# mkln/spamtree

Hardware: NVIDIA B200
Metric: mcmc_iterations_per_sec (higher is better)
Workload: dtype f64

## Files before the change

spamtree_b200/csrc/st_kernels.cu:

```cuda
#include <cuda_runtime.h>

#include <algorithm>
#include <cstdint>

#include "st_device.cuh"
#include "st_kernels.cuh"

namespace st {

__device__ __forceinline__ double iloo_term(double resid, double mean, double v, double tq) {
  const double s2 = v + 1.0 / tq, d = resid - mean;
  return -0.5 * (log(6.283185307179586 * s2) + d * d / s2);
}
template <int REF, bool ILOO>
__global__ void __launch_bounds__(kGibbsThreads)
gibbs_level_kernel(DevTree T, DevSlots D, int slot0, double* __restrict__ w, const double* __restrict__ xb,
                   const double* __restrict__ z, const double* __restrict__ tausq_inv, const double* __restrict__ SigS,
                   double* __restrict__ V, double* probe_sig, double* probe_smu, int* __restrict__ fail,
                   double* __restrict__ ll, const double* __restrict__ yobs) {
  extern __shared__ __align__(16) unsigned char smem_raw[];
  asm volatile("griddepcontrol.launch_dependents;");
  const DevSlot S = pick_slot(D, D.chain->cur);
  const int tid = threadIdx.x, nth = blockDim.x, lane = tid & 31, warp = tid >> 5;
  const int sd = slot0 + blockIdx.x;
  const int m = T.m[sd], k = T.k[sd], P = T.P[sd], coff = T.chain_off[sd], row0 = T.row0[sd];
  const int rsm = tile_rs(m), gs = T.gs[sd];
  const int msq = REF ? m * rsm : m;
  double* RiS = reinterpret_cast<double*>(smem_raw);
  double* Sig = RiS + msq;
  double* wpa = Sig + (REF ? m * m : m);
  double* gwj = wpa + P;
  double* smu = gwj + (size_t)(k + 1) * m;
  double* wn = smu + m;
  double* rr = wn + m;
  const double* G = S.G + T.goff[sd];
  const double* Rig = S.Ri + T.rioff[sd];
  const int nch = T.child_ptr[sd + 1] - T.child_ptr[sd];
  const int* ch = T.child_idx + T.child_ptr[sd];
  __shared__ int c_m[32], c_po[32], c_r0[32];
  __shared__ long long c_voff[16];
  __shared__ double cbuf[128];
  if (tid < k) {
    const int a = T.chain[coff + tid];
    c_m[tid] = T.m[a]; c_po[tid] = T.chain_poff[coff + tid]; c_r0[tid] = T.row0[a];
  }
  for (int c = tid; c < min(nch, 16); c += nth) c_voff[c] = T.voff[ch[c]];
  for (int e = tid; e < msq; e += nth) RiS[e] = Rig[e];
  if (REF) {
    const long long so0 = T.soff[sd];
    for (int e = tid; e < m * m; e += nth) Sig[e] = (so0 >= 0) ? SigS[so0 + e] : 0.0;
  }
  for (int a = tid; a < m; a += nth) {
    const double tq = tausq_inv[T.mvq[row0 + a]];
    wn[a] = tq;
    smu[a] = tq * (T.y[row0 + a] - xb[row0 + a]);
    rr[a] = z[row0 + a];
  }
  __syncthreads();
  for (int e = tid; e < P; e += nth) {
    int j = 0;
    while (j + 1 < k && e >= c_po[j + 1]) j++;
    wpa[e] = w[c_r0[j] + (e - c_po[j])];
  }
  __syncthreads();
  for (int e = tid; e < k * m; e += nth) {
    const int r = e / k, j = e - r * k;
    const int mj = c_m[j], po = c_po[j];
    const double* g = G + (size_t)r * gs + po;
    const double* wv = wpa + po;
    double s[4] = {0, 0, 0, 0};
    int pp = 0;
    for (; pp + 8 <= mj; pp += 8) {
      double x[8];
#pragma unroll
      for (int u = 0; u < 8; u++) x[u] = g[pp + u];
#pragma unroll
      for (int u = 0; u < 8; u++) s[u & 3] = fma(x[u], wv[pp + u], s[u & 3]);
    }
    if (pp + 4 <= mj) {
      double x[4];
#pragma unroll
      for (int u = 0; u < 4; u++) x[u] = g[pp + u];
#pragma unroll
      for (int u = 0; u < 4; u++) s[u] = fma(x[u], wv[pp + u], s[u]);
      pp += 4;
    }
    for (; pp < mj; pp++) s[0] = fma(g[pp], wv[pp], s[0]);
    gwj[j * m + r] = (s[0] + s[1]) + (s[2] + s[3]);
  }
  __syncthreads();
  for (int r = tid; r < m; r += nth) {
    double s = 0;
    for (int j = 0; j < k; j++) s += gwj[j * m + r];
    gwj[k * m + r] = s;
  }
  __syncthreads();
  const double* gw = gwj + (size_t)k * m;
  if (REF) {
    for (int e = tid; e < m * m; e += nth) {
      const int a = e / m, b = e - a * m;
      double s = 0;
      for (int r = max(a, b); r < m; r++) s = fma(RiS[r * rsm + a], RiS[r * rsm + b], s);
      s += Sig[e];
      if (a == b) s += wn[a];
      Sig[e] = s;
      if (probe_sig) probe_sig[T.rioff[sd] + e] = s;
    }
    __syncthreads();
    bool okc = true;
    double myinv = 0.0;
    if (warp == 0) {
      if (m <= 32) {
        double a[32];
#pragma unroll
        for (int j = 0; j < 32; j++) a[j] = (lane < m && j <= lane) ? Sig[lane * m + j] : 0.0;
        cbuf[32 + lane] = 0.0;
        cbuf[96 + lane] = 0.0;
        __syncwarp();
        for (int j = 0; j < m; j++) {
          double d = __shfl_sync(0xffffffffu, a[0], j);
          if (!(d > 0.0) || !isfinite(d)) { okc = false; d = 1.0; }
          const double inv = rsqrt(d), sd = d * inv;
          const double l = (lane == j) ? sd : ((lane > j) ? a[0] * inv : 0.0);
          if (lane == j) myinv = inv;
          if (lane >= j && lane < m) Sig[lane * m + j] = l;
          double* cc = cbuf + (j & 1) * 64;
          cc[lane] = l;
          __syncwarp();
          const double* cj = cc + j + 1;
#pragma unroll
          for (int i = 0; i < 31; i++) a[i] = fma(-l, cj[i], a[i + 1]);
          a[31] = 0.0;
        }
        __syncwarp();
      } else {
        okc = warp_chol(Sig, m, m, lane);
      }
    }
    asm volatile("griddepcontrol.wait;" ::: "memory");
    for (int a = tid; a < m; a += nth) {
      double s = 0;
      for (int r = a; r < m; r++) s = fma(RiS[r * rsm + a], gw[r], s);
      for (int c = 0; c < nch; c++) s += V[(c < 16 ? c_voff[c] : T.voff[ch[c]]) + (T.limited ? 0 : P) + a];
      s += smu[a];
      smu[a] = s;
      if (probe_smu) probe_smu[row0 + a] = s;
    }
    __syncthreads();
    if (warp == 0) {
      if (okc && m <= 32) {
        double b = (lane < m) ? smu[lane] : 0.0;
        for (int j = 0; j < m; j++) {
          const double xj = __shfl_sync(0xffffffffu, b * myinv, j);
          if (lane == j) b = xj; else if (lane > j && lane < m) b = fma(-Sig[lane * m + j], xj, b);
        }
        double y = (lane < m) ? b + rr[lane] : 0.0;
        for (int j = m - 1; j >= 0; j--) {
          const double wj = __shfl_sync(0xffffffffu, y * myinv, j);
          if (lane == j) y = wj; else if (lane < j) y = fma(-Sig[j * m + lane], wj, y);
        }
        if (lane < m) { wn[lane] = y; w[row0 + lane] = y; }
      } else if (okc) {
        for (int c = 0; c < m; c++) {
          __syncwarp();
          const double xc = smu[c] / Sig[c * m + c];
          __syncwarp();
          if (lane == 0) smu[c] = xc;
          for (int r = c + 1 + lane; r < m; r += 32) smu[r] -= Sig[r * m + c] * xc;
        }
        __syncwarp();
        for (int r = lane; r < m; r += 32) smu[r] += rr[r];
        for (int c = m - 1; c >= 0; c--) {
          __syncwarp();
          const double xc = smu[c] / Sig[c * m + c];
          __syncwarp();
          if (lane == 0) smu[c] = xc;
          for (int r = lane; r < c; r += 32) smu[r] -= Sig[c * m + r] * xc;
        }
        __syncwarp();
        for (int r = lane; r < m; r += 32) { wn[r] = smu[r]; w[row0 + r] = smu[r]; }
      }
      if (!okc) {
        if (lane == 0) atomicAdd(fail, 1);
        for (int r = lane; r < m; r += 32) wn[r] = w[row0 + r];
      }
    }
    __syncthreads();
    if (ILOO) {
      const long long so0 = T.soff[sd];
      const bool back = (m & 1) == 0;
      for (int a = tid; a < m; a += nth) {
        const int i = row0 + a;
        const double yi = yobs[i];
        if (isnan(yi)) continue;
        double lz = 0.0, qa = 0.0;
        for (int t = 0; t <= a; t++) {
          const int j = back ? a - t : t;
          lz = fma(Sig[a * m + j], rr[j], lz);
        }
        for (int r = a; r < m; r++) qa = fma(RiS[r * rsm + a], RiS[r * rsm + a], qa);
        if (so0 >= 0) qa += SigS[so0 + (long long)a * m + a];
        const double tq = tausq_inv[T.mvq[i]], res = yi - xb[i], wa = wn[a];
        ll[i] = iloo_term(res, wa - (lz + tq * (res - wa)) / qa, 1.0 / qa, tq);
      }
      __syncthreads();
    }
    for (int r = tid; r < m; r += nth) {
      double s = -gw[r];
      for (int r2 = 0; r2 <= r; r2++) s = fma(RiS[r * rsm + r2], wn[r2], s);
      rr[r] = s;
    }
  } else {
    asm volatile("griddepcontrol.wait;" ::: "memory");
    for (int a = tid; a < m; a += nth) {
      const double ri = RiS[a], prec = ri * ri;
      const double sig = prec + wn[a];
// ... 22 lines not shown
    int j = 0;
    while (j + 1 < k && e >= c_po[j + 1]) j++;
    const int rsj = gs;
    const double* g = G + e;
    const double* vj = gwj + (size_t)j * m;
    double sa[4] = {0, 0, 0, 0};
    int r = 0;
    for (; r + 8 <= m; r += 8) {
      double x[8];
#pragma unroll
      for (int u = 0; u < 8; u++) x[u] = g[(size_t)(r + u) * rsj];
#pragma unroll
      for (int u = 0; u < 8; u++) sa[u & 3] = fma(x[u], vj[r + u], sa[u & 3]);
    }
    if (r + 4 <= m) {
      double x[4];
#pragma unroll
      for (int u = 0; u < 4; u++) x[u] = g[(size_t)(r + u) * rsj];
#pragma unroll
      for (int u = 0; u < 4; u++) sa[u] = fma(x[u], vj[r + u], sa[u]);
      r += 4;
    }
    for (; r < m; r++) sa[0] = fma(g[(size_t)r * rsj], vj[r], sa[0]);
    double s = (sa[0] + sa[1]) + (sa[2] + sa[3]);
    if (!T.limited)
      for (int c = 0; c < nch; c++) s += V[(c < 16 ? c_voff[c] : T.voff[ch[c]]) + e];
    Vd[e] = s;
  }
}

cudaError_t launch_gibbs(int is_ref, const DevTree& T, const DevSlots& D, int slot0, int nslots, double* w,
                         const double* xb, const double* z, const double* tausq_inv, const double* SigS, double* V,
                         double* probe_sig, double* probe_smu, int* fail, size_t smem, cudaStream_t st, bool pdl, double* ll,
                         const double* yobs) {
  if (nslots <= 0) return cudaSuccess;
  static SmemOptIn optin[4];
  const bool iloo = ll != nullptr;
  auto kern = is_ref ? (iloo ? gibbs_level_kernel<1, true> : gibbs_level_kernel<1, false>)
                     : (iloo ? gibbs_level_kernel<0, true> : gibbs_level_kernel<0, false>);
  {
    cudaError_t e = ensure_dynamic_smem(kern, smem, optin[(is_ref ? 1 : 0) + (iloo ? 2 : 0)]);
    if (e != cudaSuccess) return e;
  }
  cudaLaunchConfig_t cfg = {};
  cfg.gridDim = dim3(nslots);
  cfg.blockDim = dim3(kGibbsThreads);
  cfg.dynamicSmemBytes = smem;
  cfg.stream = st;
  cudaLaunchAttribute attr[1];
  attr[0].id = cudaLaunchAttributeProgrammaticStreamSerialization;
  attr[0].val.programmaticStreamSerializationAllowed = 1;
  cfg.attrs = attr;
  cfg.numAttrs = pdl ? 1 : 0;
  return cudaLaunchKernelEx(&cfg, kern, T, D, slot0, w, xb, z, tausq_inv, SigS, V, probe_sig, probe_smu, fail, ll, yobs);
}

__global__ void __launch_bounds__(kGramThreads)
gram_level_kernel(DevTree T, DevSlots D, int slot0, double* __restrict__ U, double* __restrict__ SigS, int rch, int ldx,
                  int stage_off, const int* __restrict__ run_flag) {
  extern __shared__ __align__(16) double gram_smem[];
  asm volatile("griddepcontrol.launch_dependents;");
  if (run_flag != nullptr && *run_flag == 0) return;
  const DevSlot S = pick_slot(D, D.chain->cur);
  __shared__ int t_po[kMaxChain + 1], t_m[kMaxChain + 1], t_item0[kMaxChain + 2], t_uo[kMaxChain + 1], t_to[kMaxChain + 2];
  __shared__ int s_rows;
  __shared__ long long s_rowoff[kGramMaxRows];
  __shared__ int s_rowncol[kGramMaxRows];
  __shared__ long long s_cu[kGramChildTab];
  __shared__ int f_m[kGramFusedTab], f_gs[kGramFusedTab], f_r0[kGramFusedTab + 1];
  __shared__ long long f_goff[kGramFusedTab];
  const int tid = threadIdx.x, nth = blockDim.x;
  const int sd = slot0 + blockIdx.x;
  if (T.ufused[sd]) return;
  double* tiles = gram_smem;
  double* stage = gram_smem + stage_off;
  const int m = T.m[sd], k = T.k[sd], P = T.P[sd], coff = T.chain_off[sd];
  const int nch = T.child_ptr[sd + 1] - T.child_ptr[sd];
  const int* ch = T.child_idx + T.child_ptr[sd];
  const long long so = T.soff[sd];
  const int ntile = k + (so >= 0 ? 1 : 0);
  if (tid <= k) {
    t_po[tid] = (tid < k) ? T.chain_poff[coff + tid] : (T.limited ? 0 : P);
    t_m[tid] = (tid < k) ? T.m[T.chain[coff + tid]] : m;
    t_uo[tid] = (tid < k) ? T.chain_uoff[coff + tid] : 0;
  }
  const bool ftab = nch <= kGramFusedTab;
  if (ftab && tid < nch) {
// ... 1307 lines not shown
```

spamtree_b200/csrc/st_kernels.cuh:

```cuda
#pragma once
#include <cuda_runtime.h>

#include <cstddef>
#include <cstdint>

#include "st_build_plan.cuh"
#include "st_model.hpp"

namespace st {

constexpr int kGibbsThreads = 64;
constexpr int kGramThreads = 256;
constexpr int kGramMaxRows = 256;
constexpr int kGramChildTab = 256;
constexpr int kGramFusedTab = 64;
constexpr int kLlwThreads = 128;
constexpr int kLlwMaxP = 1024;
constexpr double kHl2pi = -0.91893853320467274178;

inline size_t gibbs_smem_bytes(int is_ref, int m, int P, int k) {
  const size_t msq = is_ref ? (size_t)m * tile_rs(m) + (size_t)m * m : 2 * (size_t)m;
  return 8 * (msq + (size_t)P + (size_t)(k + 1) * m + 3 * (size_t)m) + 16;
}

struct SmemOptIn { size_t configured[64] = {}; };
template <class K>
inline cudaError_t ensure_dynamic_smem(K kern, size_t smem, SmemOptIn& table) {
  int dev = 0;
  cudaError_t e = cudaGetDevice(&dev);
  if (e != cudaSuccess) return e;
  if (dev < 0 || dev >= 64) return cudaFuncSetAttribute(kern, cudaFuncAttributeMaxDynamicSharedMemorySize, (int)smem);
  if (smem <= table.configured[dev]) return cudaSuccess;
  e = cudaFuncSetAttribute(kern, cudaFuncAttributeMaxDynamicSharedMemorySize, (int)smem);
  if (e == cudaSuccess) table.configured[dev] = smem;
  return e;
}

cudaError_t launch_build(int mode, const DevTree& T, const DevSlots& D, int rel, double* predG, double* predRi, int want_H,
                         const int* grp_slot0, const int* grp_nn, int ngrp, const double* w, int* fail, int ns, int phase, size_t smem,
                         cudaStream_t st, int nthreads, unsigned long long* prof = nullptr, bool pdl = false,
                         const int* run_flag = nullptr);
cudaError_t launch_gibbs(int is_ref, const DevTree& T, const DevSlots& D, int slot0, int nslots, double* w,
                         const double* xb, const double* z, const double* tausq_inv, const double* SigS, double* V,
                         double* probe_sig, double* probe_smu, int* fail, size_t smem, cudaStream_t st, bool pdl = false,
                         double* ll = nullptr,
                         const double* yobs = nullptr);
cudaError_t launch_gram(const DevTree& T, const DevSlots& D, int slot0, int nslots, double* U, double* SigS, int rch,
                        int ldx, int tile_doubles, int stage_off, int threads, cudaStream_t st, const int* run_flag = nullptr,
                        bool pdl = false);
cudaError_t launch_llw(const DevTree& T, const DevSlots& D, int rel, int slot0, int nslots, const double* w, int maxlen, cudaStream_t st,
                       double* vrow = nullptr, int parked = 0);
constexpr int kReduceScratch = 4 * 32 + 2;
cudaError_t launch_loglik_reduce(const DevSlots& D, int rel, int n_top, int n, int* fail, double* out8, double* scratch,
                                 cudaStream_t st);
cudaError_t launch_frontier_sum(const DevTree& T, int n, const int* pseudo, const int* c0, const int* c1, const int* vlen,
                                const int* ulen, double* V, double* U, int do_v, int do_u, cudaStream_t st);
cudaError_t launch_predict_sample(const DevTree& T, int slot0, int nslots, const double* Hpred, const double* sdpred,
                                  double* w, const double* z, cudaStream_t st);
cudaError_t launch_normals(double* z, long long n, uint64_t seed, uint64_t counter, const long long* rowkey, const int* iter_ptr,
                           cudaStream_t st);
cudaError_t launch_rowstats(const DevTree& T, const int* widx, long long n_all, int p, int q, const double* w,
                            const double* xb, double* partial, int nblocks, double* out, cudaStream_t st);
cudaError_t launch_xb(const DevTree& T, long long n_all, int p, const double* bcoeff, double* xb, cudaStream_t st);
cudaError_t launch_permute(const double* src, double* dst, const long long* map, long long n, cudaStream_t st);
cudaError_t launch_crosscov(const double* x1, const double* y1, const int* q1, long long n1, const double* x2,
                            const double* y2, const int* q2, long long n2, const CovTab& tab, double* out,
                            cudaStream_t st);
cudaError_t launch_mh_propose(ChainDev* C, cudaStream_t st, int iter_offset = 0);
cudaError_t launch_mh_accept(ChainDev* C, int mode, int have_llw, cudaStream_t st, int npar = 0);
cudaError_t launch_predict_gate(ChainDev* C, cudaStream_t st);
cudaError_t launch_tausq_beta(ChainDev* C, const double* stats, const double* xtx, double* tausq_inv, double* bcoeff,
                              double* scratch, int sample_tausq, int sample_beta, cudaStream_t st, int p = 0, int q = 0);
cudaError_t launch_record(ChainDev* C, const double* tausq_inv, const double* bcoeff, double* theta_mcmc, double* beta_mcmc,
                          double* tausq_mcmc, int keep, cudaStream_t st, int tick = 0);
cudaError_t launch_yhat(const DevTree& T, const double* w, const double* xb, const double* tausq_inv, const long long* iperm,
                        const long long* rowkey, long long n, const ChainDev* C, double* out, cudaStream_t st);
cudaError_t launch_chain_tick(ChainDev* C, cudaStream_t st);
struct ThetaPack {
  int n;
// ... 41 lines not shown
```

spamtree_b200/csrc/st_model.cu:

```cuda
#include "st_model.hpp"

#include <algorithm>
#include <cmath>
#include <cstdlib>
#include <cstring>
#include <limits>
#include <numeric>

#include "../../include/spamtree_b200.h"
#include "st_kernels.cuh"

#include <chrono>
#include <dlfcn.h>
#include <nvtx3/nvToolsExt.h>

namespace st {

namespace {
struct NcclApi {
  typedef struct { char internal[128]; } UniqueId;
  int (*GetUniqueId)(UniqueId*) = nullptr;
  int (*CommInitRank)(void**, int, UniqueId, int) = nullptr;
  int (*AllReduce)(const void*, void*, size_t, int, int, void*, cudaStream_t) = nullptr;
  int (*CommDestroy)(void*) = nullptr;
// ... 447 lines not shown
        int rows = h_m[t];
        for (int c = h_child_ptr[t]; c < h_child_ptr[t + 1]; c++) if (h_ufused[h_child_idx[c]]) rows += h_m[h_child_idx[c]];
        maxrows = std::max(maxrows, rows);
        ldx = std::max(ldx, (h_P[t] + h_m[t] + 1) & ~1);
        long long td = (long long)h_m[t] * h_m[t];
        int items = ((h_m[t] + 4) / 5) * ((h_m[t] + 4) / 5 + 1) / 2;
        for (int j = 0; j < h_k[t]; j++) {
          const long long mj = h_m[h_chain[h_chain_off[t] + j]];
          td += mj * mj;
          items += (int)(((mj + 4) / 5) * ((mj + 4) / 5 + 1) / 2);
        }
        tiles = std::max(tiles, (td + 1) & ~1LL);
        maxitems = std::max(maxitems, items);
      }
      L.gram_maxrows = maxrows;
      L.gram_maxitems = maxitems;
      if (tiles * 8 > 160 * 1024) { e = "a block's message Gram tiles do not fit the Gram kernel's shared memory"; return 4; }
      L.gram_ldx = ldx;
      L.gram_tiles = (int)tiles;
      L.gram_threads = std::min(kGramThreads, std::max(64, (maxitems + 31) & ~31));
      if (L.nslots <= 2 * n_sm) L.gram_threads = kGramThreads;
      L.gram_stage_off = (maxitems <= L.gram_threads) ? 0 : (int)tiles;
      const size_t fixed = (size_t)L.gram_stage_off * 8;
      const int ctas = std::max(1, std::min(8, 65536 / (128 * L.gram_threads)));
      size_t room = (size_t)(228 - ctas) * 1024 / ctas - 9 * 1024;
      if (const char* v = getenv("ST_GRAM_ROOM")) room = (size_t)atol(v);
      room = std::max(room, std::max((size_t)tiles * 8, fixed + (size_t)ldx * 8));
      room -= fixed;
      L.gram_rch = (int)std::max<size_t>(1, std::min<size_t>(std::min(maxrows, kGramMaxRows), room / ((size_t)ldx * 8)));
    }
    return 0;
  };
  for (auto& L : levels) { int rc = make_groups(L, L.is_ref ? 0 : 1); if (rc) return rc; }
  const int early_thr = (part ? 4 : 1) * n_sm;
  n_early_levels_ = 0;
  while (n_early_levels_ + 1 < (int)levels.size() && levels[n_early_levels_].ngrp <= early_thr && !levels[n_early_levels_].deferrable)
    n_early_levels_++;
  if (!part && n_obs_nodes > 16384) n_early_levels_ = 0;
  if (const char* v = getenv("ST_EARLY_LEVELS")) n_early_levels_ = std::max(0, std::min(atoi(v), (int)levels.size() - (limited ? 1 : 0)));
  { int rc = make_groups(pred_level, 2); if (rc) return rc; }

  f_alg = f_exec = n_cov = f_alg_build = f_exec_build = b_alg_build = 0;
  for (int s = 0; s < n_obs_nodes; s++) {
    const double m = h_m[s], P = h_P[s], rho = isref[s], chi = (h_child_ptr[s + 1] > h_child_ptr[s]) ? 1.0 : 0.0;
    const double C = (double)children.len(block_of_slot[s]);
    const double fb = 2 * m * P * P + rho * (2 * m * m * P + m * m * m + 2 * m * P + 2 * m * m) + rho * chi * (m * m * P + std::pow(P + m, 3) / 3) + (1 - rho) * (4 * m * P);
    const double fg = rho * (2 * P * m * m + C * m * m + 2 * m * m * m / 3 + 2 * m * P + C * m + 4 * m * m + 2 * P * P * m + 2 * P * P + 2 * P * m) +
                      (1 - rho) * (3 * m * P + 2 * P * P * m + 2 * P * P + 2 * P * m + 10 * m);
    const double fl = 2 * m * P + rho * 2 * m * m + (1 - rho) * 2 * m;
    f_alg += fb + fg + fl;
    f_alg_build += fb;
    f_exec_build += 2 * m * P * P + rho * (2 * m * m * P + m * m * P + 2 * m * m * m / 3) + (1 - rho) * 3 * m * P + 2 * m * P;
    b_alg_build += 8 * (m * P + rho * m * m + (1 - rho) * m);
    f_exec += 2 * m * P * P + rho * (2 * m * m * P + m * m * P + 2 * m * m * m / 3) + (1 - rho) * 3 * m * P + 2 * m * P +
              (4 * m * P + rho * (2 * m * m * m / 3 + 4 * m * m)) + (2 * m * P + rho * m * m);
    n_cov += P * m + rho * m * (m + 1) / 2 + (1 - rho) * m;
  }
  return 0;
}

template <class T>
static cudaError_t dev_upload(const std::vector<T>& h, T*& d, std::vector<void*>& owned) {
  d = nullptr;
  const size_t bytes = std::max<size_t>(h.size(), 1) * sizeof(T);
  cudaError_t e = cudaMalloc((void**)&d, bytes);
  if (e != cudaSuccess) return e;
// ... 71 lines not shown
  ST_CUDA(dev_upload(h_child_idx, d_cidx, owned), "upload child_idx");
  int* d_ufused;
  ST_CUDA(dev_upload(h_ufused, d_ufused, owned), "upload ufused");
  ST_CUDA(dev_upload(h_chain, d_chain, owned), "upload chain");
  ST_CUDA(dev_upload(h_chain_poff, d_cpoff, owned), "upload chain_poff");
  ST_CUDA(dev_upload(h_chain_uoff, d_cuoff, owned), "upload chain_uoff");
  ST_CUDA(dev_upload(h_grp_slot0, d_grp_slot0, owned), "upload groups");
  ST_CUDA(dev_upload(h_grp_nn, d_grp_nn, owned), "upload groups");
  ST_CUDA(dev_upload(h_front_pseudo, d_front_pseudo, owned), "upload frontier");
  ST_CUDA(dev_upload(h_front_c0, d_front_c0, owned), "upload frontier");
  ST_CUDA(dev_upload(h_front_c1, d_front_c1, owned), "upload frontier");
  ST_CUDA(dev_upload(h_front_vlen, d_front_vlen, owned), "upload frontier");
  ST_CUDA(dev_upload(h_front_ulen, d_front_ulen, owned), "upload frontier");
  dt.cx = d_cx; dt.cy = d_cy; dt.mvq = d_mvq; dt.y = d_y; dt.X = d_X;
  dt.m = d_m; dt.row0 = d_row0; dt.isref = d_isref; dt.k = d_k; dt.P = d_P; dt.lastpar = d_lastpar; dt.chain_off = d_choff;
  dt.goff = d_goff; dt.gs = d_gs; dt.moff = d_moff; dt.limited = limited ? 1 : 0; dt.rioff = d_rioff; dt.voff = d_voff; dt.uoff = d_uoff; dt.soff = d_soff;
  dt.child_ptr = d_cptr; dt.child_idx = d_cidx; dt.ufused = d_ufused;
  dt.chain = d_chain; dt.chain_poff = d_cpoff; dt.chain_uoff = d_cuoff;
  for (int s = 0; s < 2; s++) {
    ST_CUDA(dev_zeros(ds[s].G, g_total, owned), "alloc G");
    if (keep_H) ST_CUDA(dev_zeros(ds[s].H, g_total, owned), "alloc H"); else ds[s].H = nullptr;
    ST_CUDA(dev_zeros(ds[s].Ri, ri_total, owned), "alloc Ri");
    ST_CUDA(dev_zeros(ds[s].logdet, n_obs_nodes, owned), "alloc logdet");
    ST_CUDA(dev_zeros(ds[s].llcomp, n_obs_nodes, owned), "alloc llcomp");
  }
  ST_CUDA(dev_zeros(d_w, n_all, owned), "alloc w");
  ST_CUDA(dev_zeros(d_z, n_all + 1, owned), "alloc z");
  ST_CUDA(dev_upload(xb, d_xb, owned), "upload xb");
  ST_CUDA(dev_zeros(d_V, v_total, owned), "alloc V");
  ST_CUDA(dev_zeros(d_U, u_total, owned), "alloc U");
  ST_CUDA(dev_zeros(d_S, s_total, owned), "alloc S");
  ST_CUDA(dev_zeros(d_Hpred, gpred_total, owned), "alloc Hpred");
  ST_CUDA(dev_zeros(d_sdpred, sd_total_, owned), "alloc sdpred");
  if (probes) {
    ST_CUDA(dev_zeros(d_probe_sig, ri_total, owned), "alloc probe");
    ST_CUDA(dev_zeros(d_probe_smu, n_all, owned), "alloc probe");
  }
  ST_CUDA(dev_zeros(d_scalars, 64 + kMaxStats + 1024, owned), "alloc scalars");
  rowstat_blocks_ = (int)std::min<int64_t>(592, std::max<int64_t>(1, (n_all + 255) / 256));
  ST_CUDA(dev_zeros(d_partial, (long long)rowstat_blocks_ * kMaxStats, owned), "alloc partial");
  ST_CUDA(dev_upload(Bcoeff, d_bcoeff, owned), "upload beta");
  ST_CUDA(dev_upload(tausq_inv, d_tausq_inv, owned), "upload tausq");
  {
    std::vector<int> z1(4, 0);
    ST_CUDA(dev_upload(z1, d_fail, owned), "alloc fail");
  }
  ST_CUDA(cudaMallocHost((void**)&h_scalars, (64 + kMaxStats + 1024) * sizeof(double)), "pinned scalars");
  {
    void* dc = nullptr;
    ST_CUDA(cudaMalloc(&dc, sizeof(ChainDev)), "alloc chain");
    owned.push_back(dc);
    d_mc = (ChainDev*)dc;
    ST_CUDA(cudaMallocHost((void**)&h_mc, sizeof(ChainDev)), "pinned chain");
    std::memset(h_mc, 0, sizeof(ChainDev));
    h_mc->cur = cur; h_mc->npar = (int)theta[0].size(); h_mc->p = p; h_mc->q = q;
    for (int sl = 0; sl < 2; sl++) {
      std::copy(theta[sl].begin(), theta[sl].end(), h_mc->theta[sl]);
      std::string e2;
      if (!make_covtab(theta[sl].data(), (int)theta[sl].size(), q, h_mc->tab[sl], e2)) { err = e2; return 1; }
    }
    ST_CUDA(cudaMemcpy(d_mc, h_mc, sizeof(ChainDev), cudaMemcpyHostToDevice), "upload chain");
    dslots.s[0] = ds[0]; dslots.s[1] = ds[1]; dslots.chain = d_mc;
  }
  {
    std::vector<long long> key(n_all);
    const bool pg = part && !global_rows.empty();
// ... 42 lines not shown
    }
    double* hb = h_scalars + 64 + kMaxStats;
    for (int j = 0; j < q; j++) {
      std::copy(XtX[j].a.begin(), XtX[j].a.end(), hb + (size_t)j * p * p);
      hb[q * p * p + j] = (double)nobs_by_q[j];
    }
    double* db = d_scalars + 64 + kMaxStats;
    ST_CUDA(cudaMemcpyAsync(db, hb, nx * sizeof(double), cudaMemcpyHostToDevice, stream), "H2D XtX");
    rc = allreduce_dev(db, nx);
    if (rc) { e = err; return rc; }
    ST_CUDA(cudaMemcpyAsync(hb, db, nx * sizeof(double), cudaMemcpyDeviceToHost, stream), "D2H XtX");
    ST_CUDA(cudaStreamSynchronize(stream), "sync");
    for (int j = 0; j < q; j++) {
      std::copy(hb + (size_t)j * p * p, hb + (size_t)(j + 1) * p * p, XtX[j].a.begin());
      nobs_by_q[j] = (int64_t)std::llround(hb[q * p * p + j]);
    }
  xtx_pending_ = false;
  return upload_xtx();
}

int Model::upload_xtx() {
  dvec flat((size_t)q * p * p);
  for (int j = 0; j < q; j++) std::copy(XtX[j].a.begin(), XtX[j].a.end(), flat.begin() + (size_t)j * p * p);
  ST_CUDA(cudaMemcpy(d_xtx, flat.data(), flat.size() * sizeof(double), cudaMemcpyHostToDevice), "upload XtX");
  double nb[kMaxQ] = {0};
  for (int j = 0; j < q; j++) nb[j] = (double)nobs_by_q[j];
  ST_CUDA(cudaMemcpy(d_mc->nobs, nb, sizeof(nb), cudaMemcpyHostToDevice), "upload nobs");
  return 0;
}

int Model::init(std::string& e) {
  if (const char* v = getenv("ST_BUILD_NS")) force_build_ns = atoi(v);
  if (const char* v = getenv("ST_DEFER")) defer_leaves = atoi(v) != 0;
  if (const char* v = getenv("ST_PDL")) use_pdl = atoi(v) != 0;
  if (const char* v = getenv("ST_OVERLAP")) overlap = atoi(v) != 0;
  if (const char* v = getenv("ST_LLW_OVERLAP")) llw_overlap = atoi(v) != 0;
  if (const char* v = getenv("ST_MAX_COLS")) max_group_cols = atoi(v);
  if (const char* v = getenv("ST_SMEM_BUDGET")) smem_budget = (size_t)atol(v);
  probes = keep_H;
  if (device >= 0) {
    int v = 0;
    if (cudaDeviceGetAttribute(&v, cudaDevAttrMultiProcessorCount, device) == cudaSuccess && v > 0) n_sm = v;
    else (void)cudaGetLastError();
  }
  if (spread_ctas < 0) spread_ctas = n_sm;
  if (const char* v = getenv("ST_SPREAD")) spread_ctas = atoi(v);
  int rc = build_bookkeeping(e);
  if (rc) return rc;
  if (q * (p + 1) > kMaxStats) { e = "q*(p+1) exceeds 40"; return 4; }
  rc = build_layout(e);
  if (rc) return rc;
  if (n_all >= (1LL << 31)) { e = "n_all must be below 2^31"; return 4; }
  if (device < 0) return 0;
  rc = upload(e);
  if (rc) { e = err; return rc; }
  if (part && allreduce_fn) {
    rc = partition_reduce_constants(e);
    if (rc) return rc;
  } else if (part) {
    xtx_pending_ = true;
  }
  return 0;
}

int Model::nccl_unique_id(unsigned char* out128, std::string& e) {
  NcclApi& N = nccl();
// ... 179 lines not shown
    if (part && n_top_levels >= 1 && g == n_top_levels - 1) {
      ST_CUDA(launch_frontier_sum(dt, (int)h_front_pseudo.size(), d_front_pseudo, d_front_c0, d_front_c1, d_front_vlen, d_front_ulen,
                                  d_V, d_U, 0, 1, stream), "frontier_sum_kernel");
      n_launches++;
      int rc = allreduce_dev(d_U + u_front0, u_front_len);
      if (rc) return rc;
      chained = false;
    }
    if (levels[g].gram_skip) continue;
    static const bool profile = getenv("ST_PROFILE_GIBBS") != nullptr;
    cudaEvent_t pe0 = nullptr, pe1 = nullptr;
    if (profile) { cudaEventCreate(&pe0); cudaEventCreate(&pe1); cudaEventRecord(pe0, st); }
    ST_CUDA(launch_gram(dt, dslots, levels[g].slot0, levels[g].nslots, d_U, d_S, levels[g].gram_rch, levels[g].gram_ldx, levels[g].gram_tiles,
                        levels[g].gram_stage_off, levels[g].gram_threads, st, run_flag, use_pdl && !profile && chained),
            "gram_level_kernel");
    chained = true;
    n_launches++;
    if (profile) {
      cudaEventRecord(pe1, st);
      cudaStreamSynchronize(st);
      float pms = 0;
      cudaEventElapsedTime(&pms, pe0, pe1);
      cudaEventDestroy(pe0); cudaEventDestroy(pe1);
      fprintf(stderr, "[gram profile] level slot0=%d nodes=%d rch=%d ldx=%d  %.3f ms\n", levels[g].slot0, levels[g].nslots,
              levels[g].gram_rch, levels[g].gram_ldx, pms);
    }
  }
  if (!run_flag) gram_stale = false;
  return 0;
}

int Model::gibbs_launch_only(int* fail_ptr, bool iloo) {
  NvtxRange nvtx("GIBBS");
  for (int g = (int)levels.size() - 1; g >= 0; g--) {
    const LevelInfo& L = levels[g];
    if (part && n_top_levels >= 1 && g == n_top_levels - 1) {
      ST_CUDA(launch_frontier_sum(dt, (int)h_front_pseudo.size(), d_front_pseudo, d_front_c0, d_front_c1, d_front_vlen, d_front_ulen,
                                  d_V, d_U, 1, 0, stream), "frontier_sum_kernel");
      n_launches++;
      int rc = allreduce_dev(d_V + v_front0, v_front_len);
      if (rc) return rc;
    }
    static const bool profile = getenv("ST_PROFILE_GIBBS") != nullptr;
    cudaEvent_t pe0 = nullptr, pe1 = nullptr;
    if (profile) { cudaEventCreate(&pe0); cudaEventCreate(&pe1); cudaEventRecord(pe0, stream); }
    ST_CUDA(launch_gibbs(L.is_ref, dt, dslots, L.slot0, L.nslots, d_w, d_xb, d_z, d_tausq_inv, d_S, d_V,
                         probes ? d_probe_sig : nullptr, probes ? d_probe_smu : nullptr, fail_ptr, L.smem_gibbs, stream,
                         use_pdl && !profile && g != (int)levels.size() - 1, iloo ? d_ll_int_ : nullptr,
                         iloo ? d_ll_int_ + n_all : nullptr),
            "gibbs_level_kernel");
    n_launches++;
    if (profile) {
      cudaEventRecord(pe1, stream);
      cudaStreamSynchronize(stream);
      float pms = 0;
      cudaEventElapsedTime(&pms, pe0, pe1);
      cudaEventDestroy(pe0); cudaEventDestroy(pe1);
      fprintf(stderr, "[gibbs profile] level slot0=%d nodes=%d ref=%d smem=%zu maxm=%d maxP=%d  %.3f ms\n", L.slot0, L.nslots, L.is_ref,
              L.smem_gibbs, L.maxm, L.maxP, pms);
    }
  }
  return 0;
}

int Model::deal_with_w(const double* z, uint64_t seed) {
  if (!stream) { err = "this handle has no device state (created with device < 0)"; return 2; }
  if (z) { int rc = upload_rows(z, d_z); if (rc) return rc; }
  else { int rc = draw_normals(seed); if (rc) return rc; }
  stats_valid_mode_ = -1;
  { int rc = complete_slot(cur); if (rc) return rc; }
  if (gram_stale) { int rc = refresh_grams(); if (rc) return rc; }
  const bool iloo = (keep_mask & ST_KEEP_LOGLIK_INT) != 0;
  if (iloo) { int rc = alloc_loglik_int(); if (rc) return rc; }
  ST_CUDA(cudaMemsetAsync(d_fail, 0, sizeof(int), stream), "memset");
  int rc = gibbs_launch_only(d_fail, iloo);
  if (rc) return rc;
  double* slot8 = d_scalars + 48;
  ST_CUDA(launch_loglik_reduce(dslots, 0, 0, 0, d_fail, slot8, d_red_scratch, stream), "fail count");
  if (part) { rc = allreduce_dev(slot8 + 4, 3); if (rc) return rc; }
  ST_CUDA(cudaMemcpyAsync(h_scalars + 48, slot8, 8 * sizeof(double), cudaMemcpyDeviceToHost, stream), "D2H fail");
  ST_CUDA(cudaStreamSynchronize(stream), "sync");
  if (h_scalars[48 + 6] != 0.0) { err = "Error at gibbs_sample_w: conditional precision not positive definite"; return 3; }
  if (iloo) ll_int_valid_ = true;
  return 0;
// ... 1394 lines not shown
```

spamtree_b200/csrc/st_model.hpp:

```cpp
#pragma once
#include <cuda_runtime.h>

#include <functional>
#include <initializer_list>
#include <string>
#include <vector>

#include "../../include/spamtree_b200.h"
#include "st_chain.hpp"
#include "st_common.hpp"

namespace st {

bool make_covtab(const double* theta, int n_theta, int q, CovTab& tab, std::string& err);

struct DevTree {
  const double* cx;
  const double* cy;
  const int* mvq;
  const double* y;
  const double* X;
  const int* m;
  const int* row0;
  const int* isref;
  const int* k;
  const int* P;
  const int* lastpar;
  const int* chain_off;
  const long long* goff;
  const int* gs;
  const long long* moff;
  int limited;
  const long long* rioff;
  const long long* voff;
  const long long* uoff;
  const int* ufused;
  const long long* soff;
  const int* child_ptr;
  const int* child_idx;
  const int* chain;
  const int* chain_poff;
  const int* chain_uoff;
};

struct DevSlot {
  double* G;
  double* H;
  double* Ri;
  double* logdet;
  double* llcomp;
};

struct DevSlots {
  DevSlot s[2];
  const ChainDev* chain;
};

struct LevelInfo {
  int slot0 = 0, nslots = 0;
  int is_ref = 1;
  int grp0 = 0, ngrp = 0;
  struct BuildLaunch {
    int grp0 = 0, ngrp = 0;
    size_t smem = 0;
    int threads = 128;
    int ns = 2;
  };
  std::vector<BuildLaunch> build_launches;
  bool deferrable = false;
  int maxP = 0, maxm = 0, maxNC = 0, maxk = 0;
  size_t smem_gibbs = 0;
  int gram_rch = 1, gram_ldx = 2, gram_tiles = 2, gram_stage_off = 2, gram_threads = 256;
  bool gram_skip = false;
  int gram_maxrows = 0, gram_maxitems = 0;
};

struct GroupSpec { int s, nn, NT; };

class CopyOut {
 public:
  CopyOut(cudaStream_t stream, cudaStream_t copy_stream, std::string& err) : st_(stream), cs_(copy_stream), err_(err) {}
  ~CopyOut();
  CopyOut(const CopyOut&) = delete;
  CopyOut& operator=(const CopyOut&) = delete;
  int open(std::initializer_list<double*> hosts, size_t bytes_each, int nslots, size_t n);
  double* buffer(int slot);
  int send(int slot, double* const* dst, const double* const* src, int count, size_t n);
  int finish();

 private:
// ... 25 lines not shown
  ~DrawStore() { release(); }
  int reserve(int mask, size_t bytes_each, const char* what, std::string& err);
  void commit(int mask, int64_t n, int S);
  const Store& get(int which) const { return s_[which]; }
  const Store* find(int which, const std::string& who, std::string& err) const;
  void release();
  dvec samples;

 private:
  Store s_[kStores];
};

class Model {
 public:
  ~Model();
  int64_t n_all = 0;
  int p = 0, q = 0, n_blocks = 0;
  dvec y, X, coords;
  ivec mv_id;
  CSR indexing, parents, children;
  dvec block_names, block_groups;
  ivec res_is_ref;
  bool keep_H = true;
  bool limited = false;
  int device = 0;
  size_t smem_budget = 227 * 1024 - 5 * 1024;
  int force_build_ns = 0;
  bool use_pdl = true;
  bool defer_leaves = true;
  int max_group_cols = 104;
  int n_sm = 148;
  int spread_ctas = -1;
  bool probes = true;
  int64_t n_obs = 0;
  ivec na_ix_all;
  ivec block_ct_obs, blocks_not_empty, blocks_predicting, block_is_reference;
  std::vector<ivec> u_by_block_groups;
  int n_gibbs_groups = 0, n_actual_groups = 0;
  std::vector<SmallMat> XtX;
  ivec nobs_by_q;
  int n_obs_nodes = 0, n_nodes = 0;
  std::vector<int> slot_of_block, block_of_slot;
  std::vector<int> h_m, h_row0, h_k, h_P, h_chain_off, h_chain, h_chain_poff, h_chain_uoff, h_lastpar, h_gs;
  std::vector<long long> h_goff, h_rioff, h_voff, h_uoff, h_soff, h_moff;
  std::vector<int> h_child_ptr, h_child_idx, h_ufused;
  ivec perm;
  ivec iperm;
  std::vector<LevelInfo> levels;
  LevelInfo pred_level;
  std::vector<int> h_grp_slot0, h_grp_nn;
  long long g_total = 0, ri_total = 0, v_total = 0, u_total = 0, s_total = 0, gpred_total = 0;
  bool part = false;
  int rank = 0, nranks = 1, n_top_levels = 0;
  int64_t rng_row_offset = 0, n_global_rows = 0;
  ivec global_rows;
  int (*allreduce_fn)(void*, void*, int64_t) = nullptr;
  void* allreduce_ctx = nullptr;
  int n_top_slots = 0, n_top_rows = 0, n_slots_total = 0;
  std::vector<int> h_front_pseudo, h_front_c0, h_front_c1, h_front_vlen, h_front_ulen;
  int *d_front_pseudo = nullptr, *d_front_c0 = nullptr, *d_front_c1 = nullptr, *d_front_vlen = nullptr, *d_front_ulen = nullptr;
  long long v_front0 = 0, v_front_len = 0, u_front0 = 0, u_front_len = 0;
  int allreduce_dev(double* dptr, int64_t n);
  void* nccl_comm = nullptr;
  int attach_nccl(const unsigned char* id128);
  int partition_reduce_constants(std::string& e);
  bool xtx_pending_ = false;
// ... 1 lines not shown
  int upload_xtx();
  int reduce_loglik(int rel, int* fail, double* dev_red8, double* out3_host);
  dvec theta[2];
  double loglik_w[2] = {0, 0}, logdetCi[2] = {0, 0};
  int cur = 0;
  dvec Bcoeff;
  dvec tausq_inv;
  HostRng rng;
  bool gram_stale = true;
  bool pred_H_valid = false;
  bool alter_scratch = false;
  uint64_t sweep_counter = 0;
  DevTree dt{};
  DevSlot ds[2]{};
  DevSlots dslots{};
  ChainDev *d_mc = nullptr, *h_mc = nullptr;
  long long* d_rowkey = nullptr;
  double* d_red_scratch = nullptr;
  double* d_vrow = nullptr;
  double *d_xtx = nullptr, *d_bscratch = nullptr;
  double *d_theta_mcmc = nullptr, *d_beta_mcmc = nullptr, *d_tausq_mcmc = nullptr, *d_yhat = nullptr;
  void* graph_exec_[2] = {nullptr, nullptr};
  long long graph_key_[2] = {-1, -1};
  double* d_samp_ = nullptr;
  size_t samp_cap_ = 0;
  double graph_launches_[2] = {0, 0};
  double *d_w = nullptr, *d_xb = nullptr, *d_z = nullptr, *d_V = nullptr, *d_U = nullptr, *d_S = nullptr;
  double *d_Hpred = nullptr, *d_sdpred = nullptr;
  double *d_probe_sig = nullptr, *d_probe_smu = nullptr;
  double *d_scalars = nullptr, *h_scalars = nullptr;
  double *d_partial = nullptr;
  double *d_bcoeff = nullptr, *d_tausq_inv = nullptr;
  int* d_fail = nullptr;
  int *d_grp_slot0 = nullptr, *d_grp_nn = nullptr;
  double* h_stage = nullptr;
  cudaStream_t stream = nullptr, copy_stream = nullptr;
  cudaStream_t stream2 = nullptr;
  cudaEvent_t ev_fork = nullptr, ev_join = nullptr, ev_sweep = nullptr, ev_llw = nullptr, ev_acc = nullptr, ev_cond = nullptr,
              ev_early_llw = nullptr, ev_prop = nullptr, ev_zfree = nullptr;
  cudaStream_t stream3 = nullptr;
  bool llw_overlap = false;
  bool overlap = true;
  int n_early_levels_ = 0;
  long long* d_iperm = nullptr;
  cudaEvent_t ev[14]{};
  std::vector<void*> owned;
  double n_launches = 0, f_alg = 0, f_exec = 0, n_cov = 0, f_alg_build = 0, f_exec_build = 0, b_alg_build = 0;
  std::string err;

  int init(std::string& e);
  int theta_update(int slot, const double* th);
  int get_loglik_comps_w(int slot, double* out3);
  int deal_with_w(const double* z, uint64_t seed);
  int get_loglik_w(int slot, double* out2);
  void accept_make_change();
  int predict(bool theta_changed);
  int gibbs_sample_beta(const double* zb, bool faithful_index);
  int gibbs_sample_tausq(const double* fixed);
  int get_w(double* out);
  int get_loglik_int(double* out);
  int copy_store(int which, double* out, int64_t* n_rows, int32_t* n_samples);
  int save_rows(CopyOut& co, int k, double* dev, double* host);
  int set_w(const double* in);
  int get_xb(double* out);
  int set_tausq_inv(const double* t);
  int get_node_state(int slot, int u, const std::string& which, double* out, int64_t cap, int64_t* count);
// ... 68 lines not shown
```

Baseline: 123.1.

## Precompute reference-block Cholesky factors in one parallel kernel before Gibbs sweep

Moves the formation of each reference block's posterior precision and its Cholesky factorisation out of the level-serial Gibbs sweep into a single up-front kernel that covers all reference slots at once, one warp per slot. The factors, diagonal inverses and ok flags go to global buffers, and the per-level kernels only load them. This takes dependence-free dense work off the serial level chain, with more global traffic and one extra launch as the cost. It also vectorises the in-register Cholesky update with double2 shared loads, uses 128 threads for the precomputed reference kernel, and changes when PDL is enabled for the first level launch.

Result: no change. 124.0, median of 6 (+0.7%).

```diff
diff --git a/spamtree_b200/csrc/st_kernels.cu b/spamtree_b200/csrc/st_kernels.cu
--- a/spamtree_b200/csrc/st_kernels.cu
+++ b/spamtree_b200/csrc/st_kernels.cu
@@ -12,12 +12,130 @@
   const double s2 = v + 1.0 / tq, d = resid - mean;
   return -0.5 * (log(6.283185307179586 * s2) + d * d / s2);
 }
-template <int REF, bool ILOO>
-__global__ void __launch_bounds__(kGibbsThreads)
+__device__ __forceinline__ void gibbs_form_sigma(const double* RiS, int rsm, double* Sig, const double* wn, int m, int tid, int nth,
+                                                 double* probe) {
+  for (int e = tid; e < m * m; e += nth) {
+    const int a = e / m, b = e - a * m;
+    double s = 0;
+    for (int r = max(a, b); r < m; r++) s = fma(RiS[r * rsm + a], RiS[r * rsm + b], s);
+    s += Sig[e];
+    if (a == b) s += wn[a];
+    Sig[e] = s;
+    if (probe) probe[e] = s;
+  }
+}
+__device__ __forceinline__ bool gibbs_chol_regs(double (&a)[32], double* Sig, int m, double* cbuf, int lane, double& myinv) {
+  bool okc = true;
+  cbuf[32 + lane] = 0.0;
+  cbuf[96 + lane] = 0.0;
+  __syncwarp();
+  for (int j = 0; j < m; j++) {
+    double d = __shfl_sync(0xffffffffu, a[0], j);
+    if (!(d > 0.0) || !isfinite(d)) { okc = false; d = 1.0; }
+    const double inv = rsqrt(d), sd = d * inv;
+    const double l = (lane == j) ? sd : ((lane > j) ? a[0] * inv : 0.0);
+    if (lane == j) myinv = inv;
+    if (lane >= j && lane < m) Sig[lane * m + j] = l;
+    double* cc = cbuf + (j & 1) * 64 + (~j & 1);
+    cc[lane] = l;
+    __syncwarp();
+    const double2* cj = reinterpret_cast<const double2*>(cc + j + 1);
+#pragma unroll
+    for (int i = 0; i < 15; i++) {
+      const double2 v = cj[i];
+      a[2 * i] = fma(-l, v.x, a[2 * i + 1]);
+      a[2 * i + 1] = fma(-l, v.y, a[2 * i + 2]);
+    }
+    a[30] = fma(-l, cj[15].x, a[31]);
+    a[31] = 0.0;
+  }
+  __syncwarp();
+  return okc;
+}
+__device__ __forceinline__ bool gibbs_chol(double* Sig, int m, double* cbuf, int lane, double& myinv) {
+  if (m > 32) return warp_chol(Sig, m, m, lane);
+  double a[32];
+#pragma unroll
+  for (int j = 0; j < 32; j++) a[j] = (lane < m && j <= lane) ? Sig[lane * m + j] : 0.0;
+  return gibbs_chol_regs(a, Sig, m, cbuf, lane, myinv);
+}
+
+__global__ void __launch_bounds__(kGibbsFactorWarps * 32)
+gibbs_factor_kernel(DevTree T, DevSlots D, const int* __restrict__ ref_slots, int nref, const double* __restrict__ tausq_inv,
+                    const double* __restrict__ SigS, GibbsFactor F, double* probe_sig, int* __restrict__ fail, int ws, int nw) {
+  extern __shared__ __align__(16) double gf_smem[];
+  const int lane = threadIdx.x & 31, wp = threadIdx.x >> 5;
+  const int b = blockIdx.x * nw + wp;
+  if (b >= nref) return;
+  const DevSlot S = pick_slot(D, D.chain->cur);
+  const int sd = ref_slots[b];
+  const int m = T.m[sd], row0 = T.row0[sd], rsm = tile_rs(m);
+  const long long ro = T.rioff[sd], so0 = T.soff[sd];
+  double* RiS = gf_smem + (size_t)wp * ws;
+  double* cbuf = RiS + m * rsm;
+  double* Sig = cbuf + 128;
+  double* wn = Sig + m * m;
+  const double* Rig = S.Ri + ro;
+  for (int e = lane; e < m * rsm; e += 32) RiS[e] = Rig[e];
+  for (int e = lane; e < m * m; e += 32) Sig[e] = (so0 >= 0) ? SigS[so0 + e] : 0.0;
+  for (int a = lane; a < m; a += 32) wn[a] = tausq_inv[T.mvq[row0 + a]];
+  __syncwarp();
+  double myinv = 0.0;
+  bool okc;
+  if (m <= 32) {
+    double a[32];
+#pragma unroll
+    for (int j = 0; j < 32; j++) a[j] = 0.0;
+    for (int r = 0; r < m; r++) {
+      const double* row = RiS + r * rsm;
+      const double x = (lane <= r) ? row[lane] : 0.0;
+#pragma unroll
+      for (int j = 0; j < 32; j++) {
+        if (j > r) break;
+        if (j <= lane && lane <= r) a[j] = fma(x, row[j], a[j]);
+      }
+    }
+#pragma unroll
+    for (int j = 0; j < 32; j++)
+      if (lane < m && j <= lane) {
+        a[j] += Sig[lane * m + j];
+        if (j == lane) a[j] += wn[lane];
+        if (probe_sig) { probe_sig[ro + lane * m + j] = a[j]; probe_sig[ro + j * m + lane] = a[j]; }
+      }
+    __syncwarp();
+    okc = gibbs_chol_regs(a, Sig, m, cbuf, lane, myinv);
+  } else {
+    gibbs_form_sigma(RiS, rsm, Sig, wn, m, lane, 32, probe_sig ? probe_sig + ro : nullptr);
+    __syncwarp();
+    okc = gibbs_chol(Sig, m, cbuf, lane, myinv);
+  }
+  double* Lg = F.L + ro;
+  for (int e = lane; e < m * m; e += 32) Lg[e] = Sig[e];
+  if (m <= 32 && lane < m) F.inv[row0 + lane] = myinv;
+  if (lane == 0) {
+    F.ok[sd] = okc ? 1 : 0;
+    if (!okc) atomicAdd(fail, 1);
+  }
+}
+
+cudaError_t launch_gibbs_factor(const DevTree& T, const DevSlots& D, const int* ref_slots, int nref, const double* tausq_inv,
+                                const double* SigS, const GibbsFactor& F, double* probe_sig, int* fail, int ws, cudaStream_t st) {
+  if (nref <= 0) return cudaSuccess;
+  static SmemOptIn optin;
+  const int nw = (int)std::max<size_t>(1, std::min<size_t>(kGibbsFactorWarps, 227 * 1024 / ((size_t)ws * sizeof(double))));
+  const size_t smem = (size_t)nw * ws * sizeof(double);
+  cudaError_t e = ensure_dynamic_smem(gibbs_factor_kernel, smem, optin);
+  if (e != cudaSuccess) return e;
+  gibbs_factor_kernel<<<(nref + nw - 1) / nw, nw * 32, smem, st>>>(T, D, ref_slots, nref, tausq_inv, SigS, F, probe_sig, fail, ws, nw);
+  return cudaGetLastError();
+}
+
+template <int REF, bool ILOO, bool PRE>
+__global__ void __launch_bounds__(REF && PRE ? kGibbsRefThreads : kGibbsThreads)
 gibbs_level_kernel(DevTree T, DevSlots D, int slot0, double* __restrict__ w, const double* __restrict__ xb,
                    const double* __restrict__ z, const double* __restrict__ tausq_inv, const double* __restrict__ SigS,
                    double* __restrict__ V, double* probe_sig, double* probe_smu, int* __restrict__ fail,
-                   double* __restrict__ ll, const double* __restrict__ yobs) {
+                   double* __restrict__ ll, const double* __restrict__ yobs, GibbsFactor F) {
   extern __shared__ __align__(16) unsigned char smem_raw[];
   asm volatile("griddepcontrol.launch_dependents;");
   const DevSlot S = pick_slot(D, D.chain->cur);
@@ -39,14 +157,17 @@
   const int* ch = T.child_idx + T.child_ptr[sd];
   __shared__ int c_m[32], c_po[32], c_r0[32];
   __shared__ long long c_voff[16];
-  __shared__ double cbuf[128];
+  __shared__ __align__(16) double cbuf[128];
   if (tid < k) {
     const int a = T.chain[coff + tid];
     c_m[tid] = T.m[a]; c_po[tid] = T.chain_poff[coff + tid]; c_r0[tid] = T.row0[a];
   }
   for (int c = tid; c < min(nch, 16); c += nth) c_voff[c] = T.voff[ch[c]];
   for (int e = tid; e < msq; e += nth) RiS[e] = Rig[e];
-  if (REF) {
+  if (REF && PRE) {
+    const double* Lg = F.L + T.rioff[sd];
+    for (int e = tid; e < m * m; e += nth) Sig[e] = Lg[e];
+  } else if (REF) {
     const long long so0 = T.soff[sd];
     for (int e = tid; e < m * m; e += nth) Sig[e] = (so0 >= 0) ? SigS[so0 + e] : 0.0;
   }
@@ -97,45 +218,17 @@
   __syncthreads();
   const double* gw = gwj + (size_t)k * m;
   if (REF) {
-    for (int e = tid; e < m * m; e += nth) {
-      const int a = e / m, b = e - a * m;
-      double s = 0;
-      for (int r = max(a, b); r < m; r++) s = fma(RiS[r * rsm + a], RiS[r * rsm + b], s);
-      s += Sig[e];
-      if (a == b) s += wn[a];
-      Sig[e] = s;
-      if (probe_sig) probe_sig[T.rioff[sd] + e] = s;
-    }
-    __syncthreads();
     bool okc = true;
     double myinv = 0.0;
-    if (warp == 0) {
-      if (m <= 32) {
-        double a[32];
-#pragma unroll
-        for (int j = 0; j < 32; j++) a[j] = (lane < m && j <= lane) ? Sig[lane * m + j] : 0.0;
-        cbuf[32 + lane] = 0.0;
-        cbuf[96 + lane] = 0.0;
-        __syncwarp();
-        for (int j = 0; j < m; j++) {
-          double d = __shfl_sync(0xffffffffu, a[0], j);
-          if (!(d > 0.0) || !isfinite(d)) { okc = false; d = 1.0; }
-          const double inv = rsqrt(d), sd = d * inv;
-          const double l = (lane == j) ? sd : ((lane > j) ? a[0] * inv : 0.0);
-          if (lane == j) myinv = inv;
-          if (lane >= j && lane < m) Sig[lane * m + j] = l;
-          double* cc = cbuf + (j & 1) * 64;
-          cc[lane] = l;
-          __syncwarp();
-          const double* cj = cc + j + 1;
-#pragma unroll
-          for (int i = 0; i < 31; i++) a[i] = fma(-l, cj[i], a[i + 1]);
-          a[31] = 0.0;
-        }
-        __syncwarp();
-      } else {
-        okc = warp_chol(Sig, m, m, lane);
-      }
+    if (PRE) {
+      if (warp == 0) {
+        okc = F.ok[sd] != 0;
+        if (m <= 32 && lane < m) myinv = F.inv[row0 + lane];
+      }
+    } else {
+      gibbs_form_sigma(RiS, rsm, Sig, wn, m, tid, nth, probe_sig ? probe_sig + T.rioff[sd] : nullptr);
+      __syncthreads();
+      if (warp == 0) okc = gibbs_chol(Sig, m, cbuf, lane, myinv);
     }
     asm volatile("griddepcontrol.wait;" ::: "memory");
     for (int a = tid; a < m; a += nth) {
@@ -181,7 +274,7 @@
         for (int r = lane; r < m; r += 32) { wn[r] = smu[r]; w[row0 + r] = smu[r]; }
       }
       if (!okc) {
-        if (lane == 0) atomicAdd(fail, 1);
+        if (lane == 0 && !PRE) atomicAdd(fail, 1);
         for (int r = lane; r < m; r += 32) wn[r] = w[row0 + r];
       }
     }
@@ -270,19 +363,20 @@
 cudaError_t launch_gibbs(int is_ref, const DevTree& T, const DevSlots& D, int slot0, int nslots, double* w,
                          const double* xb, const double* z, const double* tausq_inv, const double* SigS, double* V,
                          double* probe_sig, double* probe_smu, int* fail, size_t smem, cudaStream_t st, bool pdl, double* ll,
-                         const double* yobs) {
+                         const double* yobs, const GibbsFactor* F) {
   if (nslots <= 0) return cudaSuccess;
-  static SmemOptIn optin[4];
-  const bool iloo = ll != nullptr;
-  auto kern = is_ref ? (iloo ? gibbs_level_kernel<1, true> : gibbs_level_kernel<1, false>)
-                     : (iloo ? gibbs_level_kernel<0, true> : gibbs_level_kernel<0, false>);
+  static SmemOptIn optin[8];
+  const bool iloo = ll != nullptr, pre = is_ref && F != nullptr;
+  auto kern = pre ? (iloo ? gibbs_level_kernel<1, true, true> : gibbs_level_kernel<1, false, true>)
+                  : is_ref ? (iloo ? gibbs_level_kernel<1, true, false> : gibbs_level_kernel<1, false, false>)
+                           : (iloo ? gibbs_level_kernel<0, true, false> : gibbs_level_kernel<0, false, false>);
   {
-    cudaError_t e = ensure_dynamic_smem(kern, smem, optin[(is_ref ? 1 : 0) + (iloo ? 2 : 0)]);
+    cudaError_t e = ensure_dynamic_smem(kern, smem, optin[(is_ref ? 1 : 0) + (iloo ? 2 : 0) + (pre ? 4 : 0)]);
     if (e != cudaSuccess) return e;
   }
   cudaLaunchConfig_t cfg = {};
   cfg.gridDim = dim3(nslots);
-  cfg.blockDim = dim3(kGibbsThreads);
+  cfg.blockDim = dim3(pre ? kGibbsRefThreads : kGibbsThreads);
   cfg.dynamicSmemBytes = smem;
   cfg.stream = st;
   cudaLaunchAttribute attr[1];
@@ -290,7 +384,8 @@
   attr[0].val.programmaticStreamSerializationAllowed = 1;
   cfg.attrs = attr;
   cfg.numAttrs = pdl ? 1 : 0;
-  return cudaLaunchKernelEx(&cfg, kern, T, D, slot0, w, xb, z, tausq_inv, SigS, V, probe_sig, probe_smu, fail, ll, yobs);
+  const GibbsFactor f = pre ? *F : GibbsFactor{};
+  return cudaLaunchKernelEx(&cfg, kern, T, D, slot0, w, xb, z, tausq_inv, SigS, V, probe_sig, probe_smu, fail, ll, yobs, f);
 }
 
 __global__ void __launch_bounds__(kGramThreads)
diff --git a/spamtree_b200/csrc/st_kernels.cuh b/spamtree_b200/csrc/st_kernels.cuh
--- a/spamtree_b200/csrc/st_kernels.cuh
+++ b/spamtree_b200/csrc/st_kernels.cuh
@@ -10,6 +10,8 @@
 namespace st {
 
 constexpr int kGibbsThreads = 64;
+constexpr int kGibbsRefThreads = 128;
+constexpr int kGibbsFactorWarps = 1;
 constexpr int kGramThreads = 256;
 constexpr int kGramMaxRows = 256;
 constexpr int kGramChildTab = 256;
@@ -18,6 +20,7 @@
 constexpr int kLlwMaxP = 1024;
 constexpr double kHl2pi = -0.91893853320467274178;
 
+inline int gibbs_factor_warp_doubles(int m) { return m * tile_rs(m) + m * m + m + 128; }
 inline size_t gibbs_smem_bytes(int is_ref, int m, int P, int k) {
   const size_t msq = is_ref ? (size_t)m * tile_rs(m) + (size_t)m * m : 2 * (size_t)m;
   return 8 * (msq + (size_t)P + (size_t)(k + 1) * m + 3 * (size_t)m) + 16;
@@ -44,7 +47,10 @@
                          const double* xb, const double* z, const double* tausq_inv, const double* SigS, double* V,
                          double* probe_sig, double* probe_smu, int* fail, size_t smem, cudaStream_t st, bool pdl = false,
                          double* ll = nullptr,
-                         const double* yobs = nullptr);
+                         const double* yobs = nullptr,
+                         const GibbsFactor* F = nullptr);
+cudaError_t launch_gibbs_factor(const DevTree& T, const DevSlots& D, const int* ref_slots, int nref, const double* tausq_inv,
+                                const double* SigS, const GibbsFactor& F, double* probe_sig, int* fail, int ws, cudaStream_t st);
 cudaError_t launch_gram(const DevTree& T, const DevSlots& D, int slot0, int nslots, double* U, double* SigS, int rch,
                         int ldx, int tile_doubles, int stage_off, int threads, cudaStream_t st, const int* run_flag = nullptr,
                         bool pdl = false);
diff --git a/spamtree_b200/csrc/st_model.cu b/spamtree_b200/csrc/st_model.cu
--- a/spamtree_b200/csrc/st_model.cu
+++ b/spamtree_b200/csrc/st_model.cu
@@ -503,6 +503,13 @@
     return 0;
   };
   for (auto& L : levels) { int rc = make_groups(L, L.is_ref ? 0 : 1); if (rc) return rc; }
+  gfac_ws = 0;
+  std::vector<int> ref_slots;
+  for (const auto& L : levels)
+    if (L.is_ref)
+      for (int t = L.slot0; t < L.slot0 + L.nslots; t++) { ref_slots.push_back(t); gfac_ws = std::max(gfac_ws, gibbs_factor_warp_doubles(h_m[t])); }
+  n_ref_slots = (int)ref_slots.size();
+  h_ref_slots_.swap(ref_slots);
   const int early_thr = (part ? 4 : 1) * n_sm;
   n_early_levels_ = 0;
   while (n_early_levels_ + 1 < (int)levels.size() && levels[n_early_levels_].ngrp <= early_thr && !levels[n_early_levels_].deferrable)
@@ -640,6 +647,12 @@
   ST_CUDA(dev_zeros(d_S, s_total, owned), "alloc S");
   ST_CUDA(dev_zeros(d_Hpred, gpred_total, owned), "alloc Hpred");
   ST_CUDA(dev_zeros(d_sdpred, sd_total_, owned), "alloc sdpred");
+  if (gibbs_prefactor && n_ref_slots > 0) {
+    ST_CUDA(dev_upload(h_ref_slots_, d_ref_slots, owned), "upload reference slots");
+    ST_CUDA(dev_zeros(gfac_.L, ri_total, owned), "alloc Gibbs factor");
+    ST_CUDA(dev_zeros(gfac_.inv, n_all, owned), "alloc Gibbs factor");
+    ST_CUDA(dev_upload(std::vector<int>(n_slots_total, 0), gfac_.ok, owned), "alloc Gibbs factor");
+  }
   if (probes) {
     ST_CUDA(dev_zeros(d_probe_sig, ri_total, owned), "alloc probe");
     ST_CUDA(dev_zeros(d_probe_smu, n_all, owned), "alloc probe");
@@ -748,6 +761,7 @@
 int Model::init(std::string& e) {
   if (const char* v = getenv("ST_BUILD_NS")) force_build_ns = atoi(v);
   if (const char* v = getenv("ST_DEFER")) defer_leaves = atoi(v) != 0;
+  if (const char* v = getenv("ST_GIBBS_PREFACTOR")) gibbs_prefactor = atoi(v) != 0;
   if (const char* v = getenv("ST_PDL")) use_pdl = atoi(v) != 0;
   if (const char* v = getenv("ST_OVERLAP")) overlap = atoi(v) != 0;
   if (const char* v = getenv("ST_LLW_OVERLAP")) llw_overlap = atoi(v) != 0;
@@ -993,6 +1007,25 @@
 
 int Model::gibbs_launch_only(int* fail_ptr, bool iloo) {
   NvtxRange nvtx("GIBBS");
+  static const bool profile = getenv("ST_PROFILE_GIBBS") != nullptr;
+  const bool pre = gfac_.L != nullptr;
+  if (pre) {
+    cudaEvent_t pe0 = nullptr, pe1 = nullptr;
+    if (profile) { cudaEventCreate(&pe0); cudaEventCreate(&pe1); cudaEventRecord(pe0, stream); }
+    ST_CUDA(launch_gibbs_factor(dt, dslots, d_ref_slots, n_ref_slots, d_tausq_inv, d_S, gfac_, probes ? d_probe_sig : nullptr,
+                                fail_ptr, gfac_ws, stream),
+            "gibbs_factor_kernel");
+    n_launches++;
+    if (profile) {
+      cudaEventRecord(pe1, stream);
+      cudaStreamSynchronize(stream);
+      float pms = 0;
+      cudaEventElapsedTime(&pms, pe0, pe1);
+      cudaEventDestroy(pe0); cudaEventDestroy(pe1);
+      fprintf(stderr, "[gibbs profile] factor blocks=%d ws=%d  %.3f ms\n", n_ref_slots, gfac_ws, pms);
+    }
+  }
+  bool after_level = false;
   for (int g = (int)levels.size() - 1; g >= 0; g--) {
     const LevelInfo& L = levels[g];
     if (part && n_top_levels >= 1 && g == n_top_levels - 1) {
@@ -1002,15 +1035,15 @@
       int rc = allreduce_dev(d_V + v_front0, v_front_len);
       if (rc) return rc;
     }
-    static const bool profile = getenv("ST_PROFILE_GIBBS") != nullptr;
     cudaEvent_t pe0 = nullptr, pe1 = nullptr;
     if (profile) { cudaEventCreate(&pe0); cudaEventCreate(&pe1); cudaEventRecord(pe0, stream); }
     ST_CUDA(launch_gibbs(L.is_ref, dt, dslots, L.slot0, L.nslots, d_w, d_xb, d_z, d_tausq_inv, d_S, d_V,
                          probes ? d_probe_sig : nullptr, probes ? d_probe_smu : nullptr, fail_ptr, L.smem_gibbs, stream,
-                         use_pdl && !profile && g != (int)levels.size() - 1, iloo ? d_ll_int_ : nullptr,
-                         iloo ? d_ll_int_ + n_all : nullptr),
+                         use_pdl && !profile && after_level, iloo ? d_ll_int_ : nullptr,
+                         iloo ? d_ll_int_ + n_all : nullptr, pre ? &gfac_ : nullptr),
             "gibbs_level_kernel");
     n_launches++;
+    after_level = after_level || L.nslots > 0;
     if (profile) {
       cudaEventRecord(pe1, stream);
       cudaStreamSynchronize(stream);
diff --git a/spamtree_b200/csrc/st_model.hpp b/spamtree_b200/csrc/st_model.hpp
--- a/spamtree_b200/csrc/st_model.hpp
+++ b/spamtree_b200/csrc/st_model.hpp
@@ -56,6 +56,12 @@
   const ChainDev* chain;
 };
 
+struct GibbsFactor {
+  double* L;
+  double* inv;
+  int* ok;
+};
+
 struct LevelInfo {
   int slot0 = 0, nslots = 0;
   int is_ref = 1;
@@ -147,6 +153,7 @@
   int n_sm = 148;
   int spread_ctas = -1;
   bool probes = true;
+  bool gibbs_prefactor = true;
   int64_t n_obs = 0;
   ivec na_ix_all;
   ivec block_ct_obs, blocks_not_empty, blocks_predicting, block_is_reference;
@@ -214,6 +221,10 @@
   double *d_partial = nullptr;
   double *d_bcoeff = nullptr, *d_tausq_inv = nullptr;
   int* d_fail = nullptr;
+  GibbsFactor gfac_{};
+  int* d_ref_slots = nullptr;
+  int n_ref_slots = 0, gfac_ws = 0;
+  std::vector<int> h_ref_slots_;
   int *d_grp_slot0 = nullptr, *d_grp_nn = nullptr;
   double* h_stage = nullptr;
   cudaStream_t stream = nullptr, copy_stream = nullptr;
```
